# CogitatorTech/vq

Hardware: AMD Instinct MI355X
Metric: pq_encode_vectors_per_s (higher is better)
Workload: dtype f32 (bf16x3-split MFMA screen, exact f32 re-check)

## Files before the change

### vq_amd/csrc/k_screen_bf16.hip

```cpp
#include <cstdlib>

#include "kernels.hpp"

namespace vqhip {
namespace {

typedef float f32x4 __attribute__((ext_vector_type(4)));
typedef short bf16x8 __attribute__((ext_vector_type(8)));
typedef unsigned int u32x4 __attribute__((ext_vector_type(4)));

constexpr int kWavesPerBlock = 4;
constexpr int kBlock = kWavesPerBlock * 64;
constexpr uint64_t kPipeMinSteps = 8;

__host__ __device__ constexpr int pair_a(int p) { return p == 0 ? 0 : p == 1 ? 1 : p == 2 ? 0 : p == 3 ? 2 : p == 4 ? 1 : 0; }
__host__ __device__ constexpr int pair_x(int p) { return p == 0 ? 0 : p == 1 ? 0 : p == 2 ? 1 : p == 3 ? 0 : p == 4 ? 1 : 2; }

__host__ __device__ inline void split3(float v, uint32_t (&part)[3]) {
    uint32_t b0, b1, b2;
#if defined(__HIP_DEVICE_COMPILE__)
    b0 = __float_as_uint(v) & 0xFFFF0000u;
    const float r1 = v - __uint_as_float(b0);
    b1 = __float_as_uint(r1) & 0xFFFF0000u;
    const float r2 = r1 - __uint_as_float(b1);
// ... 287 lines not shown
#pragma unroll
            for (int f = 0; f < NMF; ++f) {
                u32x4 v;
#pragma unroll
                for (int w = 0; w < 4; ++w) v[w] = base[((i * NMF + f) * 4 + w) * 64];
                a[i][f] = __builtin_bit_cast(bf16x8, v);
            }
        const uint32_t c_first = grp * NT32 * 32;
        const float *pc = prepCn + (size_t)s * cn_stride + c_first;
        for (uint32_t e = lane; e < NT32 * 32; e += 64) {
            float v = (c_first + e < cn_stride) ? pc[e] : 3.0e38f;
            if (cosine) v = (c_first + e < k_real) ? 0.0f : 3.0e38f;
            lds_cn[wave][e] = (v < 3.0e38f) ? v : 3.0e38f;
        }
    }
    const f32x4 *cnp = reinterpret_cast<const f32x4 *>(&lds_cn[wave][4 * h]);
    float pinf = __builtin_inff(), ninf = -__builtin_inff();
    uint32_t idx_mask = 0xFFFFFFC0u;
    asm volatile("" : "+s"(idx_mask));
    asm volatile("" : "+s"(pinf), "+s"(ninf));
    float cmax, tcoef;
    float mu[DPH];
    if (cosine) {
        cmax = 0.0f;
        tcoef = meta[s * 4 + 3];
        if (tcoef <= 3.0e38f)
            tcoef = (6.0f * SD + 2.5f * kBf16AssumedUlps * NMF + 200.0f) * 5.9604644775390625e-08f;
#pragma unroll
        for (int q = 0; q < DPH; ++q) mu[q] = 0.0f;
    } else {
        const float *cs = cen + (size_t)s * (SD + 4);
        cmax = cs[SD];
        tcoef = cs[SD + 1];
#pragma unroll
        for (int q = 0; q < DPH; ++q) mu[q] = cs[DPH * h + q];
    }

    const size_t col0 = (size_t)s * (PVW > 0 ? sdr : (uint32_t)SD) + (size_t)DPH * h;
    const size_t sub0 = (size_t)s * (PVW > 0 ? sdr : (uint32_t)SD);
    auto load_x = [&](uint64_t row, float (&x)[DPH]) {
        if (row >= n) row = n - 1;
        const float *ptr = X + row * d + col0;
        if constexpr (PVW > 0) {
            constexpr int VW = (PVW == 4 && DPH % 4 != 0) ? 2 : PVW;
            const float *first = X + row * d + sub0;
#pragma unroll
            for (int q = 0; q < DPH; q += VW) {
                const bool live = (uint32_t)(DPH * h + q) < sdr;
                const float *pq = live ? ptr + q : first;
                if constexpr (VW == 4) {
                    const float4 t = *reinterpret_cast<const float4 *>(pq);
                    x[q + 0] = live ? t.x : 0.0f;
                    x[q + 1] = live ? t.y : 0.0f;
                    x[q + 2] = live ? t.z : 0.0f;
                    x[q + 3] = live ? t.w : 0.0f;
                } else if constexpr (VW == 2) {
                    const float2 t = *reinterpret_cast<const float2 *>(pq);
                    x[q + 0] = live ? t.x : 0.0f;
                    x[q + 1] = live ? t.y : 0.0f;
                } else {
                    const float t = *pq;
                    x[q] = live ? t : 0.0f;
                }
            }
        } else if constexpr (DPH % 4 == 0) {
#pragma unroll
            for (int q = 0; q < DPH; q += 4) {
                const float4 t = *reinterpret_cast<const float4 *>(ptr + q);
                x[q + 0] = t.x;
                x[q + 1] = t.y;
                x[q + 2] = t.z;
                x[q + 3] = t.w;
            }
        } else {
#pragma unroll
            for (int q = 0; q < DPH; q += 2) {
                const float2 t = *reinterpret_cast<const float2 *>(ptr + q);
                x[q + 0] = t.x;
                x[q + 1] = t.y;
            }
        }
    };
    auto init_acc = [&](f32x16 &acc, int i) {
#pragma unroll
        for (int q = 0; q < 4; ++q) {
            const f32x4 c4 = cnp[(32 * i + 8 * q) / 4];
            acc[4 * q + 0] = c4[0];
            acc[4 * q + 1] = c4[1];
            acc[4 * q + 2] = c4[2];
            acc[4 * q + 3] = c4[3];
        }
    };

    float xn_[DPH];
    load_x(st0 * 32 + p, xn_);
    for (uint64_t st = st0; st < st1; ++st) {
        float x[DPH];
        float xo[ACC ? DPH : 1];
#pragma unroll
        for (int q = 0; q < DPH; ++q) {
            x[q] = xn_[q] - mu[q];
            if constexpr (ACC) xo[q] = xn_[q];
        }
        if (st + 1 < st1) load_x((st + 1) * 32 + p, xn_);

        uint32_t xp[3][DPH];
        float xs = 0.0f;
#pragma unroll
        for (int q = 0; q < DPH; ++q) {
            uint32_t parts[3];
            split3(x[q], parts);
            xp[0][q] = parts[0];
            xp[1][q] = parts[1];
            xp[2][q] = parts[2];
            xs = fmaf(x[q], x[q], xs);
        }
        bf16x8 b[NMF];
#pragma unroll
        for (int f = 0; f < NMF; ++f) {
            u32x4 v;
#pragma unroll
            for (int w = 0; w < 4; ++w) {
                uint32_t hw[2];
#pragma unroll
                for (int hh = 0; hh < 2; ++hh) {
                    const int flat = 8 * f + 2 * w + hh, pair = flat / DPH, dd = flat % DPH;
                    hw[hh] = (pair < 6) ? xp[pair_x(pair)][dd] : 0u;
                }
                v[w] = (hw[0] >> 16) | (hw[1] & 0xFFFF0000u);
            }
            b[f] = __builtin_bit_cast(bf16x8, v);
        }
#pragma unroll
        for (int f = 0; f < NMF; ++f) asm volatile("" ::"v"(b[f]));
        if constexpr (ACC) {
            __builtin_amdgcn_sched_barrier(0);
            acc_issue();
            __builtin_amdgcn_sched_barrier(0);
        }

        float q1[4] = {pinf, pinf, pinf, pinf}, q2[4] = {pinf, pinf, pinf, pinf};
        f32x16 acc[4];
        auto reduce8 = [&](const f32x16 &fin, int ifin, int g8) {
#pragma unroll
            for (int r = 0; r < 4; ++r) {
                const uint32_t ca = (uint32_t)((16 * ifin + 8 * g8 + r) & 63), cb = (uint32_t)((16 * ifin + 8 * g8 + 4 + r) & 63);
                const float pa = __uint_as_float((__float_as_uint(fin[8 * g8 + r]) & idx_mask) | ca);
                const float pb = __uint_as_float((__float_as_uint(fin[8 * g8 + 4 + r]) & idx_mask) | cb);
                const float t = __builtin_amdgcn_fmed3f(q1[r], pa, pb);
                q1[r] = __builtin_fminf(__builtin_fminf(q1[r], pa), pb);
                q2[r] = __builtin_fminf(q2[r], t);
            }
        };
        auto mfma = [&](f32x16 &accv, int ti, int f) {
            if ((ti * NMF + f + 1) * 4 <= 256)
                asm volatile("v_mfma_f32_32x32x16_bf16 %0, %1, %2, %0" : "+v"(accv) : "a"(a[ti][f]), "v"(b[f]));
            else
                asm volatile("v_mfma_f32_32x32x16_bf16 %0, %1, %2, %0" : "+v"(accv) : "v"(a[ti][f]), "v"(b[f]));
        };
        float snap[4] = {pinf, pinf, pinf, pinf};
        init_acc(acc[0], 0);
        if (NT32 > 1) init_acc(acc[1], 1);
        if (NT32 > 2) init_acc(acc[2], 2);
        asm volatile("s_nop 1");
#pragma unroll
        for (int f = 0; f < NMF; ++f)
            mfma(acc[0], 0, f);
        if (NT32 > 1) {
#pragma unroll
            for (int f = 0; f < NMF; ++f)
                mfma(acc[1], 1, f);
        } else {
            asm volatile("s_nop 7\n\ts_nop 7\n\ts_nop 7" ::: "memory");
        }
        if constexpr (ACC) {
            __builtin_amdgcn_sched_barrier(0);
            acc_commit();
            __builtin_amdgcn_sched_barrier(0);
        }
#pragma unroll
        for (int i = 0; i < NT32; ++i) {
            if (i + 3 < NT32) init_acc(acc[(i + 3) & 3], i + 3);
            if (i == 4) {
#pragma unroll
                for (int r = 0; r < 4; ++r) snap[r] = q1[r];
            }
            constexpr int kGroups = 4;
            if constexpr (NMF <= 6) {
#pragma unroll
                for (int f = 0; f < (NMF > kGroups ? NMF : kGroups); ++f) {
                    if (i + 2 < NT32 && f < NMF) mfma(acc[(i + 2) & 3], (i + 2 < NT32) ? i + 2 : 0, f);
                    if (f < kGroups && (f & 1)) reduce8(acc[i & 3], i, f >> 1);
                    __builtin_amdgcn_sched_barrier(0);
                }
            } else {
#pragma unroll
                for (int f = 0; f < NMF; ++f) {
                    if (i + 2 < NT32) mfma(acc[(i + 2) & 3], (i + 2 < NT32) ? i + 2 : 0, f);
#pragma unroll
                    for (int g8 = 0; g8 < kGroups / 2; ++g8)
                        if (f == ((g8 + 1) * NMF + kGroups / 2 - 1) / (kGroups / 2) - 1) reduce8(acc[i & 3], i, g8);
                    __builtin_amdgcn_sched_barrier(0);
                }
            }
            if (i + 2 >= NT32 && i + 1 < NT32) asm volatile("s_nop 7\n\ts_nop 7" ::: "memory");
        }

        auto merge2 = [&](float a1, float a2, uint32_t ai, float b1, float b2, uint32_t bi, float &o1, float &o2,
                          uint32_t &oi) {
            const float hi = __builtin_amdgcn_fmed3f(a1, b1, pinf);
            const float lo2 = __builtin_amdgcn_fmed3f(a2, b2, ninf);
            o2 = __builtin_amdgcn_fmed3f(hi, lo2, ninf);
            const bool tb = b1 < a1;
            o1 = tb ? b1 : a1;
            oi = tb ? bi : ai;
        };
        float u1, u2, w1, w2, m1, m2;
        uint32_t ui, wi, vidx;
        uint32_t vi[4];
#pragma unroll
        for (int r = 0; r < 4; ++r)
            vi[r] = (__float_as_uint(q1[r]) & 63u) + ((NT32 > 4 && q1[r] < snap[r]) ? 64u : 0u);
        merge2(q1[0], q2[0], vi[0], q1[1], q2[1], vi[1], u1, u2, ui);
        merge2(q1[2], q2[2], vi[2], q1[3], q2[3], vi[3], w1, w2, wi);
        merge2(u1, u2, ui, w1, w2, wi, m1, m2, vidx);
        uint32_t j = ((vidx >> 4) << 5) + (vidx & 3u) + (((vidx >> 2) & 3u) << 3) + 4 * h + grp * NT32 * 32;
        {
            const auto r1 = __builtin_amdgcn_permlane32_swap(__float_as_uint(m1), __float_as_uint(m1), false, false);
            const auto r2 = __builtin_amdgcn_permlane32_swap(__float_as_uint(m2), __float_as_uint(m2), false, false);
            const auto rj = __builtin_amdgcn_permlane32_swap(j, j, false, false);
            const auto rx = __builtin_amdgcn_permlane32_swap(__float_as_uint(xs), __float_as_uint(xs), false, false);
            const float a1 = __uint_as_float(r1[0]), b1 = __uint_as_float(r1[1]);
            const float a2 = __uint_as_float(r2[0]), b2 = __uint_as_float(r2[1]);
            xs = __uint_as_float(rx[0]) + __uint_as_float(rx[1]);
            const float hi = __builtin_amdgcn_fmed3f(a1, b1, pinf);
            const float lo2 = __builtin_amdgcn_fmed3f(a2, b2, ninf);
            m2 = __builtin_amdgcn_fmed3f(lo2, hi, ninf);
            const bool take = (b1 < a1) || (b1 == a1 && rj[1] < rj[0]);
            j = take ? rj[1] : rj[0];
            m1 = take ? b1 : a1;
        }
        if constexpr (G != 1) {
            const uint64_t prow = st * 32 + p;
            if (h == 0 && prow < n)
                part[((size_t)s * groups + grp) * n + prow] =
                    make_uint4(__float_as_uint(m1), __float_as_uint(m2), j, __float_as_uint(xs));
            continue;
        }
        const float xnorm = __builtin_sqrtf(xs) * 1.000001f;
        const float xn = xnorm + cmax;
        const float bnd = cosine ? xnorm : xn * xn;
        const float T = tcoef * bnd + 1e-35f * xn + 1e-37f;
        const float gap = m2 - m1;
        bool proven = (gap > T) && (fabsf(m1) <= 3.0e38f) && (T <= 3.0e38f);
        if (cosine) proven = proven && (m1 < -T) && (xnorm > 4e-10f);
        const uint64_t row = st * 32 + p;
        const bool writer = (h == 0) && (row < n);
        if (writer) {
            if (codes_t) codes_t[(size_t)s * codes_t_pitch + row] = (uint8_t)j;
            else codes[row * m + s] = (uint8_t)j;
        }
        const bool recheck = writer && !proven;
        const unsigned long long mask = __ballot(recheck);
        if (mask != 0ull) {
            if (recheck) {
                const uint32_t rank = (uint32_t)__popcll(mask & ((1ull << lane) - 1ull));
                wl_rows[(size_t)s * wl_stride + seg_first + seg_count + rank] = (uint32_t)row;
            }
            seg_count += (uint32_t)__popcll(mask);
        }
        if constexpr (ACC) {
            pend_mine = proven && (row < n);
            pend_j = j;
#pragma unroll
            for (int q = 0; q < DPH; ++q) pend_x[q] = xo[q];
            if (VQ_ACC_EXP < 2 && pend_mine && h == 0) {
                pend_before = cnts[j];
                pend_seq = atomicAdd(&cnts[j], 1u);
            }
        }
    }
    if constexpr (ACC) {
        acc_issue();
        acc_commit();
    }
    write_partial();
    if (G == 1 && lane == 0) {
        uint32_t *sg = wl_seg + ((size_t)s * n_seg + chunk) * 2;
        sg[0] = seg_first;
        sg[1] = seg_count;
    }
}

#ifndef VQ_ACC_F64
#define VQ_ACC_F64 1
#endif
#ifndef VQ_ACC_RELOAD_PAR
#define VQ_ACC_RELOAD_PAR 0
#endif
__host__ __device__ constexpr uint32_t x32p_acc_plane_bytes(int nt32) { return (uint32_t)nt32 * 32u * 8u; }
__host__ __device__ constexpr uint32_t x32p_acc_bytes_per_wave(int sd, int nt32) {
    return (uint32_t)sd * x32p_acc_plane_bytes(nt32) + 64u + ((uint32_t)nt32 * 32u + 64u) * 4u;
}

template <int SD, int NT32, bool ACC = false, int NPR = 6, int PVW = 0>
__global__ __launch_bounds__(kBlock, x32_two_waves(SD, NT32, NPR) ? 2 : 1) void k_assign_screen_bf16_x32p(
    const float *__restrict__ X, uint64_t n, uint32_t d, uint32_t m, const uint32_t *__restrict__ prepA32,
    const float *__restrict__ prepCn, uint32_t cn_stride, const float *__restrict__ meta,
    const uint32_t *__restrict__ sub_list, uint32_t n_sub, uint8_t *__restrict__ codes, uint32_t *__restrict__ wl_rows,
    uint32_t *__restrict__ wl_seg, uint32_t n_seg, uint64_t wl_stride, int cosine, uint32_t k_real,
    const float *__restrict__ cen, const uint8_t *__restrict__ gate_active, const uint32_t *__restrict__ gate_halt,
    uint8_t *__restrict__ codes_t, uint64_t codes_t_pitch, float *__restrict__ acc_sums, uint32_t *__restrict__ acc_counts,
    uint32_t sdr) {
    static_assert(NT32 == 8 && (SD == 8 || SD == 16), "pipelined screen: 8 tiles, sub_dim 8 or 16");
    static_assert(NPR == 6 || (NPR == 3 && SD == 16 && !ACC), "three products: sub_dim 16, encode form");
    static_assert(PVW == 0 || NPR == 3, "padded rows: three-product form only");
    constexpr int DPH = SD / 2;
    constexpr int NMF = (NPR * DPH + 7) / 8;
    static_assert(NPR * DPH == 8 * NMF, "every MFMA carries one term pair (sub_dim 16) or two (sub_dim 8), no padding slots");
    constexpr bool kTwo = x32_two_waves(SD, NT32, NPR);
    const bool halted = gate_halt && *gate_halt;
    const uint32_t lane = threadIdx.x & 63;
    const uint32_t h = lane >> 5, p = lane & 31;
    const uint32_t wave = __builtin_amdgcn_readfirstlane(threadIdx.x >> 6);
    const uint32_t gw = blockIdx.x * kWavesPerBlock + wave;
    const uint32_t n_chunks = n_seg;
    if (gw >= n_chunks * n_sub) return;
    const uint32_t vv = gw % n_sub;
    const uint32_t s = sub_list[vv];
    const uint32_t chunk = gw / n_sub;
    uint32_t *const seg_hdr = wl_seg + ((size_t)s * n_seg + chunk) * 2;
    const uint32_t n32 = (uint32_t)n;
    const uint32_t n_steps = (n32 + 31) / 32;
    const uint32_t steps_per_chunk = (n_steps + n_chunks - 1) / n_chunks;
    const uint32_t st0 = chunk * steps_per_chunk;
    uint32_t st1 = st0 + steps_per_chunk;
    if (st1 > n_steps) st1 = n_steps;
    if (halted || (gate_active && !gate_active[s])) {
        if (lane == 0) seg_hdr[0] = 0u, seg_hdr[1] = 0u;
        return;
    }
    extern __shared__ __attribute__((aligned(16))) float acc_lds[];
    constexpr uint32_t R = x32_acc_copies(SD, NT32);
    constexpr uint32_t kCopy = NT32 * 32 * SD;
    float *sums = nullptr;
    uint32_t *cnts = nullptr;
#if VQ_ACC_F64
    constexpr uint32_t kPlane = x32p_acc_plane_bytes(NT32);
    char *acc_wave = nullptr;
    if constexpr (ACC) {
        acc_wave = reinterpret_cast<char *>(acc_lds) + (size_t)wave * x32p_acc_bytes_per_wave(SD, NT32);
        cnts = reinterpret_cast<uint32_t *>(acc_wave + SD * kPlane + 64);
        for (uint32_t e = lane; e < (SD * kPlane + 64) / 16; e += 64) reinterpret_cast<float4 *>(acc_wave)[e] = make_float4(0.f, 0.f, 0.f, 0.f);
        for (uint32_t e = lane; e < NT32 * 32 + 64; e += 64) cnts[e] = 0u;
    }
    auto write_partial = [&]() {
        if constexpr (ACC) {
            float *ps = acc_sums + ((size_t)chunk * n_sub + vv) * k_real * SD;
            for (uint32_t e = lane; e < k_real * SD; e += 64) {
                const uint32_t j = e / SD, t = e % SD;
                ps[e] = (float)*reinterpret_cast<const double *>(acc_wave + t * kPlane + (t >= DPH ? 64u : 0u) + j * 8u);
            }
            uint32_t *pc = acc_counts + ((size_t)chunk * n_sub + vv) * k_real;
            for (uint32_t e = lane; e < k_real; e += 64) pc[e] = cnts[e];
        }
    };
#else
    if constexpr (ACC) {
        constexpr uint32_t kPerWave = NT32 * 32 * (R * SD + 1);
        sums = acc_lds + (size_t)wave * kPerWave;
        cnts = reinterpret_cast<uint32_t *>(sums + R * kCopy);
        for (uint32_t e = lane; e < R * kCopy / 4; e += 64) reinterpret_cast<float4 *>(sums)[e] = make_float4(0.f, 0.f, 0.f, 0.f);
        for (uint32_t e = lane; e < NT32 * 32; e += 64) cnts[e] = 0u;
    }
    auto write_partial = [&]() {
        if constexpr (ACC) {
            float4 *ps = reinterpret_cast<float4 *>(acc_sums + ((size_t)chunk * n_sub + vv) * k_real * SD);
            for (uint32_t e = lane; e < k_real * SD / 4; e += 64) {
                float4 t = reinterpret_cast<const float4 *>(sums)[e];
                if constexpr (R == 2) {
                    const float4 u = reinterpret_cast<const float4 *>(sums + kCopy)[e];
                    t.x = t.x + u.x;
                    t.y = t.y + u.y;
                    t.z = t.z + u.z;
                    t.w = t.w + u.w;
                }
                ps[e] = t;
            }
            uint32_t *pc = acc_counts + ((size_t)chunk * n_sub + vv) * k_real;
            for (uint32_t e = lane; e < k_real; e += 64) pc[e] = cnts[e];
        }
    };
#endif
    if (st0 >= st1) {
        write_partial();
        if (lane == 0) seg_hdr[0] = 0u, seg_hdr[1] = 0u;
        return;
    }
    const uint32_t nst = st1 - st0;
    const uint32_t seg_first = st0 * 32;
    uint32_t seg_count = 0;

    __shared__ __attribute__((aligned(16))) float lds_cn[kWavesPerBlock][NT32 * 32];
    bf16x8 a[NT32][NMF];
    {
        const uint32_t *base = prepA32 + (size_t)s * NT32 * NMF * 4 * 64 + lane;
#pragma unroll
        for (int i = 0; i < NT32; ++i)
#pragma unroll
            for (int f = 0; f < NMF; ++f) {
                u32x4 v;
#pragma unroll
                for (int w = 0; w < 4; ++w) v[w] = base[((i * NMF + f) * 4 + w) * 64];
                a[i][f] = __builtin_bit_cast(bf16x8, v);
            }
        const float *pc = prepCn + (size_t)s * cn_stride;
        for (uint32_t e = lane; e < NT32 * 32; e += 64) {
            float v = (e < cn_stride) ? pc[e] : 3.0e38f;
            if (cosine) v = (e < k_real) ? 0.0f : 3.0e38f;
            lds_cn[wave][e] = (v < 3.0e38f) ? v : 3.0e38f;
        }
    }
    const f32x4 *cnp = reinterpret_cast<const f32x4 *>(&lds_cn[wave][4 * h]);
    float pinf = __builtin_inff(), ninf = -__builtin_inff();
    uint32_t idx_mask = 0xFFFFFFC0u;
    asm volatile("" : "+s"(idx_mask));
    asm volatile("" : "+s"(pinf), "+s"(ninf));
    float cmax, tcoef;
    float mu[DPH];
    if (cosine) {
        cmax = 0.0f;
        tcoef = meta[s * 4 + 3];
        if (tcoef <= 3.0e38f) tcoef = (6.0f * SD + 2.5f * kBf16AssumedUlps * NMF + 200.0f) * 5.9604644775390625e-08f;
#pragma unroll
        for (int q = 0; q < DPH; ++q) mu[q] = 0.0f;
    } else {
        const float *cs = cen + (size_t)s * (SD + 4);
        cmax = cs[SD];
        tcoef = cs[SD + (NPR == 3 ? 2 : 1)];
#pragma unroll
        for (int q = 0; q < DPH; ++q) mu[q] = cs[DPH * h + q];
    }
    f32x4 mu4[DPH / 4];
#pragma unroll
    for (int q = 0; q < DPH; ++q) mu4[q / 4][q % 4] = mu[q];
    const size_t sub0 = (size_t)s * (PVW > 0 ? sdr : (uint32_t)SD);
    const char *const x_base = reinterpret_cast<const char *>(X + sub0 + (size_t)DPH * h);
    const uint32_t x_pitch = d * 4;
    uint8_t *const code_base = codes_t ? codes_t + (size_t)s * codes_t_pitch : codes + s;
    const uint32_t code_stride = codes_t ? 1u : m;
    constexpr int kDeep = kTwo ? 1 : 2;
    f32x4 xn_[kDeep][DPH / 4];
    auto load_x = [&](uint32_t row, int buf) {
        row = row < n32 ? row : n32 - 1;
        const float *ptr = reinterpret_cast<const float *>(x_base + (uint64_t)row * x_pitch);
        if constexpr (PVW > 0) {
            const float *first = ptr - DPH * h;
#pragma unroll
            for (int q = 0; q < DPH; q += PVW) {
                const bool live = (uint32_t)(DPH * h + q) < sdr;
                const float *pq = live ? ptr + q : first;
                if constexpr (PVW == 4) {
                    const f32x4 t = *reinterpret_cast<const f32x4 *>(pq);
#pragma unroll
                    for (int e = 0; e < 4; ++e) xn_[buf][q / 4][e] = live ? t[e] : 0.0f;
                } else if constexpr (PVW == 2) {
                    const float2 t = *reinterpret_cast<const float2 *>(pq);
                    xn_[buf][q / 4][q % 4 + 0] = live ? t.x : 0.0f;
                    xn_[buf][q / 4][q % 4 + 1] = live ? t.y : 0.0f;
                } else {
                    const float t = *pq;
                    xn_[buf][q / 4][q % 4] = live ? t : 0.0f;
                }
            }
        } else {
#pragma unroll
            for (int q = 0; q < DPH / 4; ++q) xn_[buf][q] = *reinterpret_cast<const f32x4 *>(ptr + 4 * q);
        }
    };
    auto init_acc = [&](f32x16 &acc, int i) {
#pragma unroll
        for (int q = 0; q < 4; ++q) {
            const f32x4 c4 = cnp[(32 * i + 8 * q) / 4];
            acc[4 * q + 0] = c4[0];
            acc[4 * q + 1] = c4[1];
            acc[4 * q + 2] = c4[2];
            acc[4 * q + 3] = c4[3];
        }
    };
    constexpr int kCnV = kTwo ? 0 : (ACC ? 4 : 6);
    f32x16 cnr[kCnV > 0 ? kCnV : 1];
#pragma unroll
    for (int i = 0; i < kCnV; ++i) init_acc(cnr[i], i);
    auto mfma = [&](f32x16 &accv, int ti, int f, const bf16x8 &bv) {
        if (f == 0 && ti < kCnV) {
            asm volatile("v_mfma_f32_32x32x16_bf16 %0, %1, %2, %3" : "=&v"(accv) : "a"(a[ti][f]), "v"(bv), "v"(cnr[ti]));
            return;
        }
        if constexpr (kTwo) asm volatile("v_mfma_f32_32x32x16_bf16 %0, %1, %2, %0" : "+v"(accv) : "v"(a[ti][f]), "v"(bv));
        else asm volatile("v_mfma_f32_32x32x16_bf16 %0, %1, %2, %0" : "+v"(accv) : "a"(a[ti][f]), "v"(bv));
    };

    bf16x8 b[2][NMF];
    auto bsel = [](int f) { return (NPR == 3 && f == 1) ? 0 : f; };
    float q1[2][2], q2[2][2];
    float xc[DPH];
    uint32_t xp[3][DPH];
    float xsT = 0.0f, xsM = 0.0f, xsN = 0.0f;
    f32x16 acc[4];

    constexpr int kSplitPieces = 1 + DPH / 4 + NMF;
    auto split_piece = [&](int k, int nb, uint32_t next_step, bool anchor = false) {
        if (k == 0) {
#pragma unroll
            for (int q = 0; q < DPH / 4; ++q) {
                if constexpr (kTwo && (!ACC || VQ_ACC_F64)) {
                    f32x4 dv = xn_[nb % kDeep][q] - mu4[q];
                    asm volatile("" : "+v"(dv));
                    xc[4 * q + 0] = dv[0], xc[4 * q + 1] = dv[1], xc[4 * q + 2] = dv[2], xc[4 * q + 3] = dv[3];
                } else {
#pragma unroll
                    for (int e = 0; e < 4; ++e) {
                        xc[4 * q + e] = xn_[nb % kDeep][q][e] - mu[4 * q + e];
                        asm volatile("" ::"v"(xc[4 * q + e]));
                    }
                }
            }
            xsN = 0.0f;
            load_x(next_step * 32 + p, nb % kDeep);
            if (anchor && n32 == 0xFFFFFFFFu) {
#pragma unroll
                for (int q = 0; q < DPH / 4; ++q) asm volatile("" ::"v"(xn_[nb % kDeep][q]));
            }
        } else if (k <= DPH / 4 && NPR == 3) {
#pragma unroll
            for (int w = 2 * (k - 1); w < 2 * k; ++w) {
                const float v0 = xc[2 * w], v1 = xc[2 * w + 1];
                const uint32_t p1 = cvt_pk_bf16(v0, v1);
                const float r0 = v0 - __uint_as_float(p1 << 16), r1 = v1 - __uint_as_float(p1 & 0xFFFF0000u);
                xp[0][w] = p1;
                xp[1][w] = cvt_pk_bf16(r0, r1);
                xsN = fmaf(v0, v0, xsN);
                xsN = fmaf(v1, v1, xsN);
            }
        } else if (k <= DPH / 4) {
#pragma unroll
            for (int q = 4 * (k - 1); q < 4 * k; ++q) {
                uint32_t parts[3];
                split3(xc[q], parts);
                xp[0][q] = parts[0];
                xp[1][q] = parts[1];
                xp[2][q] = parts[2];
                xsN = fmaf(xc[q], xc[q], xsN);
            }
        } else if (NPR == 3) {
            const int f = k - 1 - DPH / 4;
            if (f != 1) {
                u32x4 v;
#pragma unroll
                for (int w = 0; w < 4; ++w) v[w] = xp[f == 0 ? 0 : 1][w];
                b[nb][f] = __builtin_bit_cast(bf16x8, v);
                asm volatile("" ::"v"(b[nb][f]));
            }
        } else {
            const int f = k - 1 - DPH / 4;
            u32x4 v;
#pragma unroll
            for (int w = 0; w < 4; ++w) {
                uint32_t hw[2];
#pragma unroll
                for (int hh = 0; hh < 2; ++hh) {
                    const int flat = 8 * f + 2 * w + hh, pair = flat / DPH, dd = flat % DPH;
                    hw[hh] = xp[pair_x(pair)][dd];
                }
                v[w] = (hw[0] >> 16) | (hw[1] & 0xFFFF0000u);
            }
            b[nb][f] = __builtin_bit_cast(bf16x8, v);
            asm volatile("" ::"v"(b[nb][f]));
        }
    };
    float ta[2];
    auto min3 = [](float x, float y, float z) { return __builtin_fminf(__builtin_fminf(x, y), z); };
    auto reduce_hg = [&](const f32x16 &fin, int ifin, int hg, int par) {
        const int g8 = hg >> 1;
        const uint32_t ca = (uint32_t)(8 * ifin + 4 * g8 + (hg & 1)), cb = ca + 2u;
#pragma unroll
        for (int c = 0; c < 2; ++c) {
            const int r = 2 * (hg & 1) + c;
            const float pa = __uint_as_float((__float_as_uint(fin[8 * g8 + r]) & idx_mask) | ca);
            const float pb = __uint_as_float((__float_as_uint(fin[8 * g8 + 4 + r]) & idx_mask) | cb);
            const float t = __builtin_amdgcn_fmed3f(q1[par][c], pa, pb);
            q1[par][c] = min3(q1[par][c], pa, pb);
            if ((hg & 1) == 0) {
                ta[c] = t;
                asm volatile("" ::"v"(q1[par][c]), "v"(ta[c]));
            } else {
                q2[par][c] = min3(q2[par][c], ta[c], t);
                asm volatile("" ::"v"(q1[par][c]), "v"(q2[par][c]));
            }
        }
    };
    float t_m1 = 0.0f, t_m2 = 0.0f, t_xs = 0.0f;
    uint32_t t_j = 0;
    bool t_proven = false;
    bool pend_mine = false;
    uint32_t pend_j = 0, pend_before = 0, pend_seq = 0, pend_rank = 0xFFFFFFFFu;
    float pend_x[ACC ? DPH : 1];
    f32x4 pend_t[ACC ? DPH / 4 : 1];
    float4 *pend_slot = nullptr;
    auto acc_reload = [&](uint32_t tst) {
        if constexpr (ACC) {
            uint32_t row = tst * 32 + p;
            row = row < n32 ? row : n32 - 1;
            const float *ptr = reinterpret_cast<const float *>(x_base + (uint64_t)row * x_pitch);
#pragma unroll
            for (int q = 0; q < DPH; q += 4) {
                const float4 t = *reinterpret_cast<const float4 *>(ptr + q);
                pend_x[q + 0] = t.x;
                pend_x[q + 1] = t.y;
                pend_x[q + 2] = t.z;
                pend_x[q + 3] = t.w;
            }
        }
    };
    auto acc_ticket = [&](bool mine) {
        if constexpr (ACC) {
#if VQ_ACC_F64
            if (mine) {
                const uint32_t a0 = (uint32_t)(uintptr_t)(acc_wave) + (DPH * kPlane + 64u) * h + t_j * 8u;
                const uint32_t ac = (uint32_t)(uintptr_t)(cnts) + (h ? (NT32 * 32u + p) * 4u : t_j * 4u);
                const uint32_t one = 1u;
#pragma unroll
                for (int q = 0; q < DPH; ++q) {
                    const double v = (double)pend_x[q];
                    asm volatile("ds_add_f64 %0, %1 offset:%2" ::"v"(a0), "v"(v), "n"(q * (int)kPlane) : "memory");
                }
                asm volatile("ds_add_u32 %0, %1" ::"v"(ac), "v"(one) : "memory");
            }
            (void)pend_mine, (void)pend_j, (void)pend_before, (void)pend_seq;
#else
            pend_mine = mine;
            pend_j = t_j;
            if (pend_mine && h == 0) {
                pend_before = cnts[pend_j];
                pend_seq = atomicAdd(&cnts[pend_j], 1u);
            }
#endif
        }
    };
    auto acc_issue = [&]() {
        if constexpr (ACC && !VQ_ACC_F64) {
            uint32_t rank = (pend_mine && h == 0) ? pend_seq - pend_before : 0xFFFFFFFFu;
            rank = __builtin_amdgcn_permlane32_swap(rank, rank, false, false)[0];
            pend_rank = rank;
            const uint32_t copy = (R == 2 && rank == 1u) ? kCopy : 0u;
            pend_slot = reinterpret_cast<float4 *>(__builtin_assume_aligned(sums + copy + (size_t)(pend_mine ? pend_j : 0u) * SD + DPH * h, 16));
#pragma unroll
            for (int q = 0; q < DPH / 4; ++q) pend_t[q] = reinterpret_cast<const f32x4 *>(pend_slot)[q];
        }
    };
    auto acc_commit = [&]() {
        if constexpr (ACC && !VQ_ACC_F64) {
            if (pend_rank < R) {
#pragma unroll
                for (int q = 0; q < DPH / 4; ++q) {
                    f32x4 t = pend_t[q];
                    t[0] = t[0] + pend_x[4 * q + 0];
                    t[1] = t[1] + pend_x[4 * q + 1];
                    t[2] = t[2] + pend_x[4 * q + 2];
                    t[3] = t[3] + pend_x[4 * q + 3];
                    reinterpret_cast<f32x4 *>(pend_slot)[q] = t;
                }
            }
            for (uint32_t r = R;; ++r) {
                if (!__any(pend_rank != 0xFFFFFFFFu && pend_rank >= r)) break;
                if (pend_rank == r) {
#pragma unroll
                    for (int q = 0; q < DPH / 4; ++q) {
                        float4 t = pend_slot[q];
                        t.x = t.x + pend_x[4 * q + 0];
                        t.y = t.y + pend_x[4 * q + 1];
                        t.z = t.z + pend_x[4 * q + 2];
                        t.w = t.w + pend_x[4 * q + 3];
                        pend_slot[q] = t;
                    }
                }
                __builtin_amdgcn_wave_barrier();
            }
            pend_mine = false;
            pend_rank = 0xFFFFFFFFu;
        }
    };
    constexpr bool kAccPair = ACC && VQ_ACC_F64;
    float pend_xr[kAccPair ? SD : 1];
    auto acc_reload_pair = [&](uint32_t S) {
        if constexpr (kAccPair) {
            uint32_t row = (S - 1 + h) * 32 + p;
            row = row < n32 ? row : n32 - 1;
            const float *ptr = reinterpret_cast<const float *>(reinterpret_cast<const char *>(X + (size_t)s * SD) + (uint64_t)row * x_pitch);
            const float *pa = ptr + DPH * h, *pb = ptr - DPH * h;
#pragma unroll
            for (int q = 0; q < SD; q += 4) {
                const float4 t = *reinterpret_cast<const float4 *>((q < DPH ? pa : pb) + q);
                pend_xr[q + 0] = t.x;
                pend_xr[q + 1] = t.y;
                pend_xr[q + 2] = t.z;
                pend_xr[q + 3] = t.w;
            }
        }
    };
    constexpr int kAccPieces = SD / 4;
    bool upd_mine = false;
    uint32_t upd_j = 0;
    auto acc_update_begin = [&](bool mine) {
        if constexpr (kAccPair) upd_mine = mine, upd_j = t_j;
    };
    auto acc_update_piece = [&](int k) {
#if VQ_ACC_F64
        if constexpr (kAccPair) {
#ifdef VQ_ACC_ABL
            if (VQ_ACC_ABL == 1) return;
#endif
            if (upd_mine) {
                const uint32_t base = (uint32_t)(uintptr_t)(acc_wave) + upd_j * 8u;
                if (k < kAccPieces) {
                    const uint32_t a0 = base + ((4 * k < DPH) ? (DPH * kPlane + 64u) * h : (DPH * kPlane + 64u) * (1u - h));
#pragma unroll
                    for (int q = 4 * k; q < 4 * k + 4; ++q) {
                        const double v = (double)pend_xr[q];
                        asm volatile("ds_add_f64 %0, %1 offset:%2" ::"v"(a0), "v"(v), "n"((q < DPH ? q : q - DPH) * (int)kPlane) : "memory");
                    }
                } else {
                    const uint32_t ac = (uint32_t)(uintptr_t)(cnts) + upd_j * 4u;
                    const uint32_t one = 1u;
                    asm volatile("ds_add_u32 %0, %1" ::"v"(ac), "v"(one) : "memory");
                }
            }
        }
#endif
    };
    auto tail_piece = [&](int k, int tp, uint32_t tst, bool in_loop, bool no_step = false) {
        if (k == 0) {
            const float a1 = q1[tp][0], a2 = q2[tp][0], b1 = q1[tp][1], b2 = q2[tp][1];
            const float hi = __builtin_amdgcn_fmed3f(a1, b1, pinf);
            const float lo2 = __builtin_amdgcn_fmed3f(a2, b2, ninf);
            t_m2 = __builtin_amdgcn_fmed3f(hi, lo2, ninf);
            const bool tb = b1 < a1;
            t_m1 = tb ? b1 : a1;
            const uint32_t tag = __float_as_uint(t_m1) & 63u;
            t_j = ((tag & 62u) << 2) + ((tag & 1u) << 1) + (tb ? 1u : 0u) + 4 * h;
#pragma unroll
            for (int c = 0; c < 2; ++c) q1[tp][c] = pinf, q2[tp][c] = pinf;
        } else if (k == 1) {
            const auto r1 = __builtin_amdgcn_permlane32_swap(__float_as_uint(t_m1), __float_as_uint(t_m1), false, false);
            const auto r2 = __builtin_amdgcn_permlane32_swap(__float_as_uint(t_m2), __float_as_uint(t_m2), false, false);
            const auto rj = __builtin_amdgcn_permlane32_swap(t_j, t_j, false, false);
            const auto rx = __builtin_amdgcn_permlane32_swap(__float_as_uint(xsT), __float_as_uint(xsT), false, false);
            const float a1 = __uint_as_float(r1[0]), b1 = __uint_as_float(r1[1]);
            const float a2 = __uint_as_float(r2[0]), b2 = __uint_as_float(r2[1]);
            t_xs = __uint_as_float(rx[0]) + __uint_as_float(rx[1]);
            const float hi = __builtin_amdgcn_fmed3f(a1, b1, pinf);
            const float lo2 = __builtin_amdgcn_fmed3f(a2, b2, ninf);
            t_m2 = __builtin_amdgcn_fmed3f(lo2, hi, ninf);
            const bool take = (b1 < a1) || (b1 == a1 && rj[1] < rj[0]);
            t_j = take ? rj[1] : rj[0];
            t_m1 = take ? b1 : a1;
        } else if (k == 2) {
            const float xnorm = __builtin_sqrtf(t_xs) * 1.000001f;
            const float xn = xnorm + cmax;
            const float bnd = cosine ? xnorm : xn * xn;
            const float T = tcoef * bnd + 1e-35f * xn + 1e-37f;
            const float gap = t_m2 - t_m1;
            bool proven = (gap > T) && (fabsf(t_m1) <= 3.0e38f) && (T <= 3.0e38f);
            if (cosine) proven = proven && (t_m1 < -T) && (xnorm > 4e-10f);
            t_proven = proven;
        } else {
            const bool valid = in_loop ? !no_step : (tst < st1);
            const uint32_t row = (in_loop && !valid ? st0 : tst) * 32 + p;
            const uint32_t rowc = row < n32 ? row : n32 - 1;
            if (in_loop || valid) code_base[(uint64_t)rowc * code_stride] = (uint8_t)t_j;
            const bool writer = (h == 0) && (row < n32) && valid;
            const bool recheck = writer && !t_proven;
            const unsigned long long mask = __ballot(recheck);
            if (mask != 0ull) {
                if (recheck) {
                    const uint32_t rank = (uint32_t)__popcll(mask & ((1ull << lane) - 1ull));
                    wl_rows[(size_t)s * wl_stride + seg_first + seg_count + rank] = (uint32_t)row;
                }
                seg_count += (uint32_t)__popcll(mask);
            }
            acc_ticket(t_proven && valid && (row < n32));
        }
    };

    float held_m1 = 0.0f, held_m2 = 0.0f, held_xs = 0.0f;
    uint32_t held_j = 0;
    auto tail_hold = [&]() { held_m1 = t_m1, held_m2 = t_m2, held_j = t_j, held_xs = xsT; };
    auto tail_pair_piece = [&](int k, uint32_t S, bool first) {
        if (k == 1) {
            const auto r1 = __builtin_amdgcn_permlane32_swap(__float_as_uint(held_m1), __float_as_uint(t_m1), false, false);
            const auto r2 = __builtin_amdgcn_permlane32_swap(__float_as_uint(held_m2), __float_as_uint(t_m2), false, false);
            const auto rj = __builtin_amdgcn_permlane32_swap(held_j, t_j, false, false);
            const auto rx = __builtin_amdgcn_permlane32_swap(__float_as_uint(held_xs), __float_as_uint(xsT), false, false);
            const float a1 = __uint_as_float(r1[0]), b1 = __uint_as_float(r1[1]);
            const float a2 = __uint_as_float(r2[0]), b2 = __uint_as_float(r2[1]);
            t_xs = __uint_as_float(rx[0]) + __uint_as_float(rx[1]);
            const float hi = __builtin_amdgcn_fmed3f(a1, b1, pinf);
            const float lo2 = __builtin_amdgcn_fmed3f(a2, b2, ninf);
            t_m2 = __builtin_amdgcn_fmed3f(lo2, hi, ninf);
            const bool take = (b1 < a1) || (b1 == a1 && rj[1] < rj[0]);
            t_j = take ? rj[1] : rj[0];
            t_m1 = take ? b1 : a1;
        } else {
            const bool valid = (h != 0) || !first;
            const uint32_t row = (S - 1 + h) * 32 + p;
            uint32_t srow = row, sj = t_j;
            if (first) {
                sj = __builtin_amdgcn_permlane32_swap(t_j, t_j, false, false)[1];
                srow = S * 32 + p;
            }
            const uint32_t rowc = srow < n32 ? srow : n32 - 1;
            code_base[(uint64_t)rowc * code_stride] = (uint8_t)sj;
            const bool recheck = valid && (row < n32) && !t_proven;
            const unsigned long long mask = __ballot(recheck);
            if (mask != 0ull) {
                if (recheck) {
                    const uint32_t rank = (uint32_t)__popcll(mask & ((1ull << lane) - 1ull));
                    wl_rows[(size_t)s * wl_stride + seg_first + seg_count + rank] = (uint32_t)row;
                }
                seg_count += (uint32_t)__popcll(mask);
            }
            acc_update_begin(valid && (row < n32) && t_proven);
        }
    };

    load_x(st0 * 32 + p, 0);
    if (kDeep == 2) load_x((st0 + 1) * 32 + p, 1);
#pragma unroll
    for (int k = 0; k < kSplitPieces; ++k) split_piece(k, 0, st0 + kDeep);
    xsM = xsN;
#pragma unroll
    for (int c = 0; c < 2; ++c) q1[0][c] = q2[0][c] = q1[1][c] = q2[1][c] = pinf;
    if (0 >= kCnV) init_acc(acc[0], 0);
    if (1 >= kCnV) init_acc(acc[1], 1);
    if (2 >= kCnV) init_acc(acc[2], 2);
    asm volatile("s_nop 1");
#pragma unroll
    for (int f = 0; f < NMF; ++f) mfma(acc[0], 0, f, b[0][bsel(f)]);
#pragma unroll
    for (int f = 0; f < NMF; ++f) mfma(acc[1], 1, f, b[0][bsel(f)]);
    __builtin_amdgcn_sched_barrier(0);

#pragma clang loop unroll(full)
    for (int peel = 0; peel < 2; ++peel) {
      const bool first = peel == 0;
      for (uint32_t it0 = first ? 0u : 2u; it0 < (first ? 1u : nst); it0 += 2) {
#pragma unroll
        for (int par = 0; par < 2; ++par) {
            const uint32_t st = st0 + it0 + par;
#pragma unroll
            for (int i = 0; i < NT32; ++i) {
                if ((i + 3) % NT32 >= kCnV) init_acc(acc[(i + 3) & 3], (i + 3) % NT32);
#pragma unroll
                for (int f = 0; f < NMF; ++f) {
                    if (i + 2 < NT32) mfma(acc[(i + 2) & 3], i + 2, f, b[par][bsel(f)]);
                    else mfma(acc[(i + 2) & 3], i + 2 - NT32, f, b[par ^ 1][bsel(f)]);
                    if constexpr (NMF == 6) {
                        if (f == 0) reduce_hg(acc[i & 3], i, 0, par);
                        if (f == 1) reduce_hg(acc[i & 3], i, 1, par);
                        if (f == 3) reduce_hg(acc[i & 3], i, 2, par);
                        if (f == 4) reduce_hg(acc[i & 3], i, 3, par);
                        if (f == 2 || f == 5) {
                            const int slot = 2 * i + (f == 5);
                            if (slot == 0) {
                                if constexpr (kAccPair) { if (par == VQ_ACC_RELOAD_PAR) acc_reload_pair(st - VQ_ACC_RELOAD_PAR); }
                                else acc_reload(st - 1);
                                split_piece(0, par ^ 1, st + 1 + kDeep, first);
                            } else if (slot <= 4) {
                                if constexpr (ACC && !kAccPair) {
                                    tail_piece(slot - 1, par ^ 1, st - 1, true, first && par == 0);
                                } else if (par == 0) {
                                    if (slot == 1) tail_piece(0, 1, st - 1, true), tail_hold();
                                } else {
                                    if (slot == 1) tail_piece(0, 0, st - 1, true);
                                    else if (slot == 3) tail_piece(2, 0, st - 1, true);
                                    else tail_pair_piece(slot - 1, st - 1, first);
                                }
                            }
                            else if (slot <= 10) split_piece(slot - 4, par ^ 1, st + 1 + kDeep);
                            else if (slot == 11) split_piece(7, par ^ 1, st + 1 + kDeep), split_piece(8, par ^ 1, st + 1 + kDeep);
                            else if (slot == 12) { if constexpr (!kAccPair) acc_issue(); }
                            else if (slot == 14) { if constexpr (!kAccPair) acc_commit(); }
                            if constexpr (kAccPair) {
                                if (par == 1 && slot >= 5 && slot < 5 + kAccPieces) acc_update_piece(slot - 5);
                                if (par == 1 && slot == 5 + kAccPieces) acc_update_piece(kAccPieces);
                            }
                        }
                    } else {
                        if (f == 0) reduce_hg(acc[i & 3], i, 0, par), reduce_hg(acc[i & 3], i, 1, par);
                        if (f == 1) reduce_hg(acc[i & 3], i, 2, par), reduce_hg(acc[i & 3], i, 3, par);
                        if (f == 2) {
                            if (i == 0) {
                                if constexpr (kAccPair) { if (par == VQ_ACC_RELOAD_PAR) acc_reload_pair(st - VQ_ACC_RELOAD_PAR); }
                                else acc_reload(st - 1);
                                split_piece(0, par ^ 1, st + 1 + kDeep, first);
                                tail_piece(0, par ^ 1, st - 1, true);
                                if constexpr (ACC && !kAccPair) tail_piece(1, par ^ 1, st - 1, true, first && par == 0);
                                else if (par == 0) tail_hold();
                                else tail_pair_piece(1, st - 1, first);
                            } else if (i == 1) {
                                if constexpr (ACC && !kAccPair) tail_piece(2, par ^ 1, st - 1, true), tail_piece(3, par ^ 1, st - 1, true, first && par == 0);
                                else if (par == 1) tail_piece(2, 0, st - 1, true), tail_pair_piece(3, st - 1, first);
                                split_piece(1, par ^ 1, st + 1 + kDeep);
                            } else if (i < kSplitPieces) {
                                split_piece(i, par ^ 1, st + 1 + kDeep);
                            } else if (i == 6) {
                                if constexpr (!kAccPair) acc_issue();
                            } else if (i == 7) {
                                if constexpr (!kAccPair) acc_commit();
                            }
                            if constexpr (kAccPair) {
                                if (par == 1 && i >= 5 && i < 5 + kAccPieces) acc_update_piece(i - 5);
                                if (par == 1 && i == 5 + kAccPieces) acc_update_piece(kAccPieces);
                            }
                        }
                    }
                    __builtin_amdgcn_sched_barrier(0);
                }
            }
            xsT = xsM;
            xsM = xsN;
        }
      }
    }
    {
        const uint32_t last = st0 + ((nst + 1) & ~1u) - 1;
        acc_reload(last);
#pragma unroll
        for (int k = 0; k < 4; ++k) tail_piece(k, 1, last, false);
        acc_issue();
        acc_commit();
        write_partial();
    }
    if (lane == 0) seg_hdr[0] = seg_first, seg_hdr[1] = seg_count;
}

template <int G>
__global__ __launch_bounds__(256) void k_merge_partials_x32(const uint4 *__restrict__ part, uint64_t n, uint32_t m,
                                                            uint32_t sd, const uint32_t *__restrict__ sub_list,
                                                            const float *__restrict__ cen, const float *__restrict__ meta,
                                                            int cosine, uint8_t *__restrict__ codes,
                                                            uint32_t *__restrict__ wl_rows, uint32_t *__restrict__ wl_count,
                                                            uint64_t wl_stride, uint32_t k, uint32_t groups_rt) {
    const uint32_t groups = (G > 0) ? (uint32_t)G : groups_rt;
    const uint32_t s = sub_list[blockIdx.y];
    const float *cs = cen + (size_t)s * (sd + 4);
    float cmax = cs[sd], tcoef = cs[sd + 1];
    if (cosine) {
        const float nmf = (float)((6 * (sd / 2) + 7) / 8);
        cmax = 0.0f;
        tcoef = (meta[s * 4 + 3] <= 3.0e38f) ? (6.0f * (float)sd + 2.5f * kBf16AssumedUlps * nmf + 200.0f) * 5.9604644775390625e-08f
                                             : __builtin_inff();
    }
    const uint32_t lane = threadIdx.x & 63;
    for (uint64_t row0 = (uint64_t)blockIdx.x * 256; row0 < n; row0 += (uint64_t)gridDim.x * 256) {
        const uint64_t row = row0 + threadIdx.x;
        bool recheck = false;
        if (row < n) {
            const uint4 p0 = part[((size_t)s * groups) * n + row];
            float m1 = __uint_as_float(p0.x), m2 = __uint_as_float(p0.y);
            uint32_t j = p0.z;
            const float xs = __uint_as_float(p0.w);
#pragma unroll
            for (uint32_t g = 1; g < groups; ++g) {
                const uint4 pg = part[((size_t)s * groups + g) * n + row];
                const float b1 = __uint_as_float(pg.x), b2 = __uint_as_float(pg.y);
                const float hi = fmaxf(m1, b1), lo2 = fminf(m2, b2);
                const bool take = (b1 < m1) || (b1 == m1 && pg.z < j);
                m2 = fminf(hi, lo2);
                j = take ? pg.z : j;
                m1 = take ? b1 : m1;
            }
            const float xnorm = __builtin_sqrtf(xs) * 1.000001f;
            const float xn = xnorm + cmax;
            const float T = tcoef * (cosine ? xnorm : xn * xn) + 1e-35f * xn + 1e-37f;
            bool proven = (m2 - m1 > T) && (fabsf(m1) <= 3.0e38f) && (T <= 3.0e38f);
            if (cosine) proven = proven && (m1 < -T) && (xnorm > 4e-10f);
            store_code(codes, row * m + s, j, k);
            recheck = !proven;
        }
        const unsigned long long mask = __ballot(recheck);
        if (mask != 0ull) {
            uint32_t base = 0;
            if (lane == 0) base = atomicAdd(&wl_count[s], (uint32_t)__popcll(mask));
            base = __builtin_amdgcn_readfirstlane(base);
            if (recheck) wl_rows[(size_t)s * wl_stride + base + (uint32_t)__popcll(mask & ((1ull << lane) - 1ull))] = (uint32_t)row;
        }
    }
}

template <int NCH>
__global__ __launch_bounds__(kBlock, 1) void k_assign_screen_bf16_wide(
    const float *__restrict__ X, uint64_t n, uint32_t d, const uint32_t *__restrict__ prepA, size_t chunk_stride,
    const float *__restrict__ prepCn, uint32_t cn_stride, const uint32_t *__restrict__ sub_list, uint32_t n_sub,
    int cosine, uint32_t k_real, const float *__restrict__ cen, uint4 *__restrict__ part, uint32_t groups,
    uint32_t sdr) {
    constexpr int DPH = 32, NMF = 24, SDP = 64 * NCH;
    const uint32_t lane = threadIdx.x & 63;
    const uint32_t h = lane >> 5, p = lane & 31;
    const uint32_t wave = __builtin_amdgcn_readfirstlane(threadIdx.x >> 6);
    const uint32_t gw = blockIdx.x * kWavesPerBlock + wave;
    const uint32_t total_waves = gridDim.x * kWavesPerBlock;
    const uint32_t n_virt = n_sub * groups;
    const uint32_t n_chunks = total_waves / n_virt;
    if (gw >= n_chunks * n_virt) return;
    const uint32_t vv = gw % n_virt;
    const uint32_t s = sub_list[vv / groups];
    const uint32_t grp = vv % groups;
    const uint32_t chunk = gw / n_virt;
    const uint64_t n_steps = (n + 31) / 32;
    const uint64_t steps_per_chunk = (n_steps + n_chunks - 1) / n_chunks;
    const uint64_t st0 = (uint64_t)chunk * steps_per_chunk;
    uint64_t st1 = st0 + steps_per_chunk;
    if (st1 > n_steps) st1 = n_steps;
    if (st0 >= st1) return;

    bf16x8 a[NCH][NMF];
#pragma unroll
    for (int c = 0; c < NCH; ++c) {
        const uint32_t *base = prepA + (size_t)c * chunk_stride + ((size_t)s * groups + grp) * NMF * 4 * 64 + lane;
#pragma unroll
        for (int f = 0; f < NMF; ++f) {
            u32x4 v;
#pragma unroll
            for (int w = 0; w < 4; ++w) v[w] = base[(f * 4 + w) * 64];
            a[c][f] = __builtin_bit_cast(bf16x8, v);
        }
    }
    float cnv[16];
#pragma unroll
    for (int r = 0; r < 16; ++r) {
        const uint32_t idx = grp * 32 + (r & 3) + 8 * (r >> 2) + 4 * h;
        float v = (idx < cn_stride) ? prepCn[(size_t)s * cn_stride + idx] : 3.0e38f;
        if (cosine) v = (idx < k_real) ? 0.0f : 3.0e38f;
        cnv[r] = (v < 3.0e38f) ? v : 3.0e38f;
    }
    const float *cs = cen + (size_t)s * (SDP + 4);
    const float pinf = __builtin_inff(), ninf = -__builtin_inff();
    const size_t sub0 = (size_t)s * sdr;

    for (uint64_t st = st0; st < st1; ++st) {
        uint64_t row = st * 32 + p;
        if (row >= n) row = n - 1;
        const float *xrow = X + row * d + sub0;
        f32x16 acc;
#pragma unroll
        for (int r = 0; r < 16; ++r) acc[r] = cnv[r];
        float xs = 0.0f;
#pragma unroll
        for (int c = 0; c < NCH; ++c) {
            float x[DPH];
#pragma unroll
            for (int q = 0; q < DPH; q += 4) {
                const uint32_t dim = 64 * c + DPH * h + q;
                const bool live = dim < sdr;
                const float4 t = *reinterpret_cast<const float4 *>(xrow + (live ? dim : 0u));
                float4 mu4 = make_float4(0.f, 0.f, 0.f, 0.f);
                if (!cosine) mu4 = *reinterpret_cast<const float4 *>(cs + dim);
                x[q + 0] = live ? t.x - mu4.x : 0.0f;
                x[q + 1] = live ? t.y - mu4.y : 0.0f;
                x[q + 2] = live ? t.z - mu4.z : 0.0f;
                x[q + 3] = live ? t.w - mu4.w : 0.0f;
            }
            uint32_t xp[3][DPH];
#pragma unroll
            for (int q = 0; q < DPH; ++q) {
                uint32_t parts[3];
                split3(x[q], parts);
                xp[0][q] = parts[0];
                xp[1][q] = parts[1];
                xp[2][q] = parts[2];
                xs = fmaf(x[q], x[q], xs);
            }
#pragma unroll
            for (int f = 0; f < NMF; ++f) {
                u32x4 v;
#pragma unroll
                for (int w = 0; w < 4; ++w) {
                    uint32_t hw[2];
#pragma unroll
                    for (int hh = 0; hh < 2; ++hh) {
                        const int flat = 8 * f + 2 * w + hh, pair = flat / DPH, dd = flat % DPH;
                        hw[hh] = xp[pair_x(pair)][dd];
                    }
                    v[w] = (hw[0] >> 16) | (hw[1] & 0xFFFF0000u);
                }
                acc = __builtin_amdgcn_mfma_f32_32x32x16_bf16(a[c][f], __builtin_bit_cast(bf16x8, v), acc, 0, 0, 0);
            }
        }
        float m1 = pinf, m2 = pinf;
        uint32_t ji = 0;
#pragma unroll
        for (int r = 0; r < 16; ++r) {
            const float v = acc[r];
            const uint32_t idx = (r & 3) + 8 * (r >> 2) + 4 * h;
            m2 = __builtin_amdgcn_fmed3f(m1, m2, v);
            const bool take = (v < m1) || (v == m1 && idx < ji);
            ji = take ? idx : ji;
            m1 = take ? v : m1;
        }
        uint32_t j = grp * 32 + ji;
        {
            const auto r1 = __builtin_amdgcn_permlane32_swap(__float_as_uint(m1), __float_as_uint(m1), false, false);
            const auto r2 = __builtin_amdgcn_permlane32_swap(__float_as_uint(m2), __float_as_uint(m2), false, false);
            const auto rj = __builtin_amdgcn_permlane32_swap(j, j, false, false);
            const auto rx = __builtin_amdgcn_permlane32_swap(__float_as_uint(xs), __float_as_uint(xs), false, false);
            const float a1 = __uint_as_float(r1[0]), b1 = __uint_as_float(r1[1]);
            const float a2 = __uint_as_float(r2[0]), b2 = __uint_as_float(r2[1]);
            xs = __uint_as_float(rx[0]) + __uint_as_float(rx[1]);
            const float hi = __builtin_amdgcn_fmed3f(a1, b1, pinf);
            const float lo2 = __builtin_amdgcn_fmed3f(a2, b2, ninf);
            m2 = __builtin_amdgcn_fmed3f(lo2, hi, ninf);
            const bool take = (b1 < a1) || (b1 == a1 && rj[1] < rj[0]);
            j = take ? rj[1] : rj[0];
            m1 = take ? b1 : a1;
        }
        const uint64_t prow = st * 32 + p;
        if (h == 0 && prow < n)
            part[((size_t)s * groups + grp) * n + prow] = make_uint4(__float_as_uint(m1), __float_as_uint(m2), j, __float_as_uint(xs));
    }
}

__global__ __launch_bounds__(256) void k_codes_transpose(const uint8_t *__restrict__ ct, uint64_t pitch, uint8_t *__restrict__ codes,
                                                         uint64_t n, uint32_t m, const uint32_t *__restrict__ sub_list,
                                                         uint32_t n_sub, const uint8_t *__restrict__ gate_active,
                                                         const uint32_t *__restrict__ gate_halt) {
    extern __shared__ __attribute__((aligned(16))) uint8_t tr_lds[];
    if (gate_halt && *gate_halt) return;
    const uint32_t tp = codes_transpose_pitch(m);
    uint8_t *tile = tr_lds, *act = tr_lds + 256 * tp;
    const uint64_t row0 = (uint64_t)blockIdx.x * 256;
    for (uint32_t s = threadIdx.x; s < m; s += 256) act[s] = 0;
    __syncthreads();
    for (uint32_t i = threadIdx.x; i < n_sub; i += 256) {
        const uint32_t s = sub_list[i];
        act[s] = gate_active ? gate_active[s] : (uint8_t)1;
    }
    __syncthreads();
    const uint32_t wave = threadIdx.x >> 6, lane = threadIdx.x & 63;
    for (uint32_t s0 = wave; s0 < m; s0 += 32) {
        uint32_t v[8];
#pragma unroll
        for (uint32_t u = 0; u < 8; ++u) {
            const uint32_t s = min(s0 + 4 * u, m - 1u);
            v[u] = *reinterpret_cast<const uint32_t *>(ct + (size_t)s * pitch + row0 + 4 * lane);
        }
#pragma unroll
        for (uint32_t u = 0; u < 8; ++u) {
            const uint32_t s = s0 + 4 * u;
            if (s >= m) break;
            uint32_t w = v[u];
            if (!act[s]) {
                w = 0;
#pragma unroll
                for (uint32_t i = 0; i < 4; ++i) {
                    const uint64_t r = row0 + 4 * lane + i;
                    if (r < n) w |= (uint32_t)codes[r * m + s] << (8 * i);
                }
            }
#pragma unroll
            for (uint32_t i = 0; i < 4; ++i) tile[(4 * lane + i) * tp + s] = (uint8_t)(w >> (8 * i));
        }
    }
    __syncthreads();
    const uint32_t rows_here = (uint32_t)min((uint64_t)256, n - row0), qpr = m / 4;
    uint32_t *out = reinterpret_cast<uint32_t *>(codes + row0 * m);
    for (uint32_t idx = threadIdx.x; idx < rows_here * qpr; idx += 256) {
        const uint32_t r = idx / qpr, q = idx - r * qpr;
        out[idx] = *reinterpret_cast<const uint32_t *>(tile + r * tp + 4 * q);
    }
}

template <int SD, int NT32, int G = 1, int PVW = 0, bool ACC = false>
int launch_one_x32(const CodebookView &cb, const AssignArgs &a, hipStream_t stream, uint32_t groups_rt = 0) {
    const uint32_t groups = (G > 0) ? (uint32_t)G : groups_rt;
    const uint64_t n_steps = (a.n + 31) / 32;
    static const bool pipe_on = [] {
        const char *e = std::getenv("VQHIP_SCREEN_PIPE");
        return !(e && e[0] == '0');
    }();
    bool use3 = false;
    if constexpr (G == 1 && SD == 16 && NT32 == 8 && !ACC && PVW != 4)
        use3 = pipe_on && a.encode && cb.prepA32_3 && a.metric != VQHIP_COSINE && n_steps >= kPipeMinSteps && a.n < 0xFFFFFFC0ull;
    a.products = use3 ? 3u : 6u;
    const uint32_t waves_per_simd = (use3 || x32_two_waves(SD, NT32)) ? 2 : 1;
    const uint32_t n_virt = a.n_sub * groups;
    const uint32_t n_virt_geom = (ACC && G == 1) ? cb.m * groups : n_virt;
    uint64_t want_waves = (uint64_t)num_cus() * kWavesPerBlock * waves_per_simd;
    const uint64_t max_useful = (ACC ? std::max<uint64_t>(1, n_steps / 8) : n_steps) * n_virt_geom;
    if (want_waves > max_useful) want_waves = max_useful;
    if (want_waves < n_virt_geom) want_waves = n_virt_geom;
    uint32_t blocks = (uint32_t)((want_waves + kWavesPerBlock - 1) / kWavesPerBlock);
    while ((uint64_t)blocks * kWavesPerBlock < n_virt_geom) ++blocks;
    uint32_t n_chunks = (blocks * kWavesPerBlock) / n_virt_geom;
// ... 283 lines not shown
```

Measured before the change: 3.515 billion.

## Replace per-hg top-2 reduction with row/column grid reduction in pipelined screen

Adds a grid-based reduction for the screen distances. It keeps per-column minima across tiles and per-row tagged minima with a running top-2, then folds these into the best index and second-best value at the end of each step, instead of tracking top-2 per half-group with med3 chains. The aim is to cut the VALU min/med3 work in the MFMA shadow gaps. In exchange it adds column-minimum registers and relies on tag bit packing to reconstruct the winning index, which is easy to get wrong. The new path is on by default for sub_dim 8 and for the three-product form.

New measurement: 3.974 billion, median of 6. 1.13x the previous value.

```diff
diff --git a/vq_amd/csrc/k_screen_bf16.hip b/vq_amd/csrc/k_screen_bf16.hip
--- a/vq_amd/csrc/k_screen_bf16.hip
+++ b/vq_amd/csrc/k_screen_bf16.hip
@@ -613,8 +613,13 @@
 __host__ __device__ constexpr uint32_t x32p_acc_bytes_per_wave(int sd, int nt32) {
     return (uint32_t)sd * x32p_acc_plane_bytes(nt32) + 64u + ((uint32_t)nt32 * 32u + 64u) * 4u;
 }
-
-template <int SD, int NT32, bool ACC = false, int NPR = 6, int PVW = 0>
+__host__ __device__ constexpr int x32p_grid_cols(int sd, bool acc, int npr, int pvw) {
+    if (npr == 3) return pvw == 2 ? 0 : 8;
+    if (sd == 8) return acc ? 4 : 8;
+    return 0;
+}
+
+template <int SD, int NT32, bool ACC = false, int NPR = 6, int PVW = 0, int NC = x32p_grid_cols(SD, ACC, NPR, PVW)>
 __global__ __launch_bounds__(kBlock, x32_two_waves(SD, NT32, NPR) ? 2 : 1) void k_assign_screen_bf16_x32p(
     const float *__restrict__ X, uint64_t n, uint32_t d, uint32_t m, const uint32_t *__restrict__ prepA32,
     const float *__restrict__ prepCn, uint32_t cn_stride, const float *__restrict__ meta,
@@ -911,6 +916,82 @@
             }
         }
     };
+    static_assert(NC == 0 || ((NC == 8 || NC == 4) && NMF == 3), "grid reduce: 8 or 4 column classes, two reduce gaps per phase");
+    float cm[NC > 0 ? NC : 1];
+    float rq1 = 0.0f, rq2 = 0.0f;
+    float p_m1 = pinf, p_m2 = pinf;
+    uint32_t p_j = 0;
+    auto med3 = [](float x, float y, float z) { return __builtin_amdgcn_fmed3f(x, y, z); };
+    auto tagged = [&](float v, uint32_t tag) { return __uint_as_float((__float_as_uint(v) & idx_mask) | tag); };
+    auto reduce_grid = [&](const f32x16 &fin, int ifin, int hf) {
+        if constexpr (NC == 8) {
+#pragma unroll
+            for (int c = 4 * hf; c < 4 * hf + 4; ++c) {
+                cm[c] = ifin == 0 ? min3(fin[c], fin[c + 8], pinf) : min3(cm[c], fin[c], fin[c + 8]);
+                asm volatile("" ::"v"(cm[c]));
+            }
+            float r = min3(fin[8 * hf], fin[8 * hf + 1], fin[8 * hf + 2]);
+            r = min3(r, fin[8 * hf + 3], fin[8 * hf + 4]);
+            r = min3(r, fin[8 * hf + 5], fin[8 * hf + 6]);
+            r = min3(r, fin[8 * hf + 7], pinf);
+            const float pr = tagged(r, (uint32_t)(2 * ifin + hf));
+            if (hf == 0) {
+                ta[0] = pr;
+                asm volatile("" ::"v"(ta[0]));
+            } else {
+                const float t = med3(ifin == 0 ? pinf : rq1, ta[0], pr);
+                rq1 = min3(ifin == 0 ? pinf : rq1, ta[0], pr);
+                rq2 = ifin == 0 ? t : min3(rq2, t, pinf);
+                asm volatile("" ::"v"(rq1), "v"(rq2));
+            }
+        } else if constexpr (NC == 4) {
+#pragma unroll
+            for (int c = 0; c < 4; ++c) {
+                cm[c] = (ifin == 0 && hf == 0) ? min3(fin[c], fin[c + 4], pinf) : min3(cm[c], fin[8 * hf + c], fin[8 * hf + 4 + c]);
+                asm volatile("" ::"v"(cm[c]));
+            }
+            float pr[2];
+#pragma unroll
+            for (int w = 0; w < 2; ++w) {
+                float r = min3(fin[8 * hf + 4 * w], fin[8 * hf + 4 * w + 1], fin[8 * hf + 4 * w + 2]);
+                r = min3(r, fin[8 * hf + 4 * w + 3], pinf);
+                pr[w] = tagged(r, (uint32_t)(4 * ifin + 2 * hf + w));
+            }
+            const bool fresh = ifin == 0 && hf == 0;
+            const float t = med3(fresh ? pinf : rq1, pr[0], pr[1]);
+            rq1 = min3(fresh ? pinf : rq1, pr[0], pr[1]);
+            if (hf == 0) {
+                ta[0] = t;
+                asm volatile("" ::"v"(rq1), "v"(ta[0]));
+            } else {
+                rq2 = min3(ifin == 0 ? pinf : rq2, ta[0], t);
+                asm volatile("" ::"v"(rq1), "v"(rq2));
+            }
+        }
+    };
+    const uint32_t h4 = 4 * h;
+    auto fold_step = [&]() {
+        if constexpr (NC > 0) {
+            float pc[NC];
+#pragma unroll
+            for (int c = 0; c < NC; ++c) pc[c] = tagged(cm[c], (uint32_t)(8 * (c >> 2) + (c & 3)));
+            float c1 = min3(pc[0], pc[1], pinf), c2 = med3(pc[0], pc[1], pinf);
+            float t1 = med3(c1, pc[2], pc[3]);
+            c1 = min3(c1, pc[2], pc[3]);
+            if constexpr (NC == 8) {
+                const float t2 = med3(c1, pc[4], pc[5]);
+                c1 = min3(c1, pc[4], pc[5]);
+                c2 = min3(c2, t1, t2);
+                t1 = med3(c1, pc[6], pc[7]);
+                c1 = min3(c1, pc[6], pc[7]);
+            }
+            p_m2 = min3(c2, t1, rq2);
+            p_m1 = rq1;
+            const uint32_t cj = (__float_as_uint(c1) & 11u) | h4;
+            p_j = ((__float_as_uint(rq1) & (NC == 8 ? 15u : 31u)) << (NC == 8 ? 4 : 3)) | cj;
+            asm volatile("" ::"v"(p_m1), "v"(p_m2), "v"(p_j));
+        }
+    };
     float t_m1 = 0.0f, t_m2 = 0.0f, t_xs = 0.0f;
     uint32_t t_j = 0;
     bool t_proven = false;
@@ -1051,7 +1132,9 @@
 #endif
     };
     auto tail_piece = [&](int k, int tp, uint32_t tst, bool in_loop, bool no_step = false) {
-        if (k == 0) {
+        if (k == 0 && NC > 0) {
+            t_m1 = p_m1, t_m2 = p_m2, t_j = p_j;
+        } else if (k == 0) {
             const float a1 = q1[tp][0], a2 = q2[tp][0], b1 = q1[tp][1], b2 = q2[tp][1];
             const float hi = __builtin_amdgcn_fmed3f(a1, b1, pinf);
             const float lo2 = __builtin_amdgcn_fmed3f(a2, b2, ninf);
@@ -1208,9 +1291,14 @@
                             }
                         }
                     } else {
-                        if (f == 0) reduce_hg(acc[i & 3], i, 0, par), reduce_hg(acc[i & 3], i, 1, par);
-                        if (f == 1) reduce_hg(acc[i & 3], i, 2, par), reduce_hg(acc[i & 3], i, 3, par);
+                        if constexpr (NC > 0) {
+                            if (f < 2) reduce_grid(acc[i & 3], i, f);
+                        } else {
+                            if (f == 0) reduce_hg(acc[i & 3], i, 0, par), reduce_hg(acc[i & 3], i, 1, par);
+                            if (f == 1) reduce_hg(acc[i & 3], i, 2, par), reduce_hg(acc[i & 3], i, 3, par);
+                        }
                         if (f == 2) {
+                            if (i == NT32 - 1) fold_step();
                             if (i == 0) {
                                 if constexpr (kAccPair) { if (par == VQ_ACC_RELOAD_PAR) acc_reload_pair(st - VQ_ACC_RELOAD_PAR); }
                                 else acc_reload(st - 1);
```
